# markokr/libacm

Hardware: AMD Instinct MI355X
Metric: decoded PCM Msamples/sec over a batch of ACM streams (hot path on HBM-resident staged input) (higher is better)
Workload: dtype int32

## Files before the change

libacm_amd/csrc/acm_kernel_geo.cpp:

```cpp
#include <stdlib.h>

#include "acm_kernel_geo.h"
#include "acm_parse_bounds.h"

using namespace acm_geo;

namespace {

inline int cus_of(int cus) { return cus > 0 ? cus : 256; }
inline int switch_of(const char *text, int unset) { return text ? atoi(text) : unset; }

inline const FusedTile *fused_at(uint32_t level, int variant)
{
	if (level < ACM_K1_MIN_LEVEL || level > ACM_K1_MAX_LEVEL || variant < 0 || variant >= NVARIANTS)
		return nullptr;
	return &FUSED[variant][level - ACM_K1_MIN_LEVEL];
}

const Tile2MTile *tile2m_at(uint32_t level, int *g0 = nullptr)
{
	if (level < ACM_K2M_MIN_LEVEL || level > ACM_K2M_MAX_LEVEL)
		return nullptr;
	static const bool k3 = switch_of(ACM_TUNING_ENV("ACM_K3"), 1) != 0;
	static const int forced = switch_of(ACM_TUNING_ENV("ACM_K2M_G0"), 0);
// ... 105 lines not shown

extern "C" int acmk_tile2m_stages(uint32_t level)
{
	int g0 = 0;
	return tile2m_at(level, &g0) ? g0 : 0;
}

extern "C" int acmk_tile2m_lead_in(uint32_t level)
{
	const Tile2MTile *m = tile2m_at(level);
	return m && m->t.nt ? m->lead_in : 1;
}

extern "C" int acmk_tile2m_run_waves(uint32_t level, int cus)
{
	const Tile2MTile *m = tile2m_at(level);
	return m && m->chunk ? cus_of(cus) * m->t.w * (m->t.nt / 64) : 0;
}

extern "C" int acmk_tile2m_grid(uint32_t level, int cus)
{
	const Tile2MTile *m = tile2m_at(level);
	return m ? cus_of(cus) * m->t.w : 0;
}

#define ACM_CLAIM_MIN_PER 32u
#ifndef ACM_CLAIM_DEFAULTS
#define ACM_CLAIM_DEFAULTS { 16, 900 }, { 16, 800 }, { 16, 800 }, { 16, 800 }, { 16, 900 }
#endif
static const struct { int run_chunks, static_permille; } g_claim_default[5] = { ACM_CLAIM_DEFAULTS };
static int g_claim_run_chunks = -1, g_claim_static_permille = -1;

extern "C" int acmk_tile2m_split(uint32_t level, int cus, uint32_t ntiles, uint32_t *static_per, uint32_t *run_chunks, uint32_t *nclaimed)
{
	const uint32_t W = (uint32_t)acmk_tile2m_run_waves(level, cus);
	if (!W)
		return -1;
	const bool set = g_claim_run_chunks >= 0 || g_claim_static_permille >= 0;
	const uint32_t R = (uint32_t)(g_claim_run_chunks >= 0 ? g_claim_run_chunks : g_claim_default[level - 8].run_chunks);
	uint32_t share = (uint32_t)(g_claim_static_permille >= 0 ? g_claim_static_permille : g_claim_default[level - 8].static_permille);
	if (share > 1000u)
		share = 1000u;
	*static_per = (ntiles + W - 1) / W;
	*run_chunks = *nclaimed = 0;
	if (!R || ntiles < (set ? (uint32_t)acmk_tile2m_grid(level, cus) : W * ACM_CLAIM_MIN_PER))
		return 0;
// ... 69 lines not shown
```

libacm_amd/csrc/acm_kernel_geo.h:

```cpp
#ifndef ACM_KERNEL_GEO_H
#define ACM_KERNEL_GEO_H

#include <stdint.h>

#include <initializer_list>

#include "acm_device.h"

#if defined(ACM_ABLATION) && !defined(ACM_TUNING)
#define ACM_TUNING 1
#endif

namespace acm_geo {

template <int L_, int NT_, int NELEM_>
struct TileCfg {
	static constexpr int L = L_;
	static constexpr int NT = NT_;
	static constexpr int NELEM = NELEM_;
	static constexpr int COLS = 1 << L_;
	static constexpr int TR = NELEM_ / COLS;
	static constexpr int NJ_LAST = NELEM_ / NT_;
	static constexpr int PS = NJ_LAST >= 64 ? 6 : 5;
	static_assert(NJ_LAST == 64 || NJ_LAST == 32 || NJ_LAST == 128, "walk length of the last pass");
	static_assert(TR >= 1, "whole rows");
	static constexpr bool ROW_PAIRS = TR >= 2 && (TR % 2) == 0;
};

struct Tile { int nt, nelem, w; };
struct Launch { int threads, tile_rows, wg_per_cu; };
constexpr Launch launch_of(const Tile t, const int level) { return Launch{ t.nt, t.nt ? t.nelem >> level : 0, t.w }; }

struct FusedTile { Tile t; bool carry = false; };
#ifdef ACM_ABLATION
constexpr int NVARIANTS = 20;
#elif defined(ACM_TUNING)
constexpr int NVARIANTS = 10;
#else
constexpr int NVARIANTS = 1;
#endif
constexpr FusedTile FUSED[NVARIANTS][ACM_K1_MAX_LEVEL - ACM_K1_MIN_LEVEL + 1] = {
	{ { { 128, 8192, 2 }, true }, { { 256, 16384, 2 }, true }, { { 256, 16384, 2 }, true }, { { 256, 16384, 2 }, true }, { { 256, 16384, 2 }, true },
	  { { 256, 16384, 2 }, true }, { { 512, 32768, 2 }, true }, { { 512, 32768, 2 }, true } },
#ifdef ACM_TUNING
	{ { { 128, 8192, 2 } }, { { 512, 16384, 4 } }, { { 512, 16384, 4 } }, { { 512, 16384, 4 } }, { { 512, 16384, 4 } }, { { 512, 32768, 2 } }, { { 512, 32768, 2 } } },
	{ { { 128, 8192, 2 } }, { { 512, 32768, 2 } }, { { 512, 32768, 2 } }, { { 512, 32768, 2 } }, { { 512, 32768, 2 } }, { { 512, 32768, 2 } }, { { 512, 32768, 2 } } },
// ... 26 lines not shown
constexpr FusedTile PLANE = { { 512, 32768, 2 }, true };
struct PlaneBuild {
	using C = TileCfg<12, PLANE.t.nt, PLANE.t.nelem>;
	static constexpr int W = PLANE.t.w;
};

constexpr Tile TILE2[ACM_K2_MAX_LEVEL - ACM_K2_MIN_LEVEL + 1] = {
	{ 256, 8192, 4 }, { 256, 8192, 4 }, { 256, 8192, 4 }, { 256, 8192, 4 }, { 256, 8192, 4 }, { 256, 8192, 4 },
	{ 512, 16384, 2 },
	{ 1024, 32768, 1 },
	{ 1024, 32768, 1 },
};
template <int L_, int NT_, int NELEM_, int WPC_>
struct TileBuildOf {
	using C = TileCfg<L_, NT_, NELEM_>;
	static constexpr int WPC = WPC_, W = WPC_ * NT_ / 256;
};
template <int L_>
struct Tile2Build : TileBuildOf<L_, TILE2[L_ - ACM_K2_MIN_LEVEL].nt, TILE2[L_ - ACM_K2_MIN_LEVEL].nelem, TILE2[L_ - ACM_K2_MIN_LEVEL].w> {};

#ifndef ACM_K3_DPP_HISTORY
#define ACM_K3_DPP_HISTORY 1
#endif
template <int L_>
struct ChunkGeo {
	static constexpr int NELEM = (1 << L_) > 2048 ? (1 << L_) : 2048;
	using C = TileCfg<L_, 64, NELEM>;
	static constexpr int NW = 32768 / NELEM;
	static constexpr int L = L_, COLS = C::COLS, TR = C::TR, PS = C::PS;
	static constexpr int G = 6, QN = 1 << G, SIGMA = COLS / QN;
	static_assert(SIGMA >= 2 && TR >= 1, "sixteen instances per matrix instruction: sixteen classes of one row, or all the classes of 2 / 4 / 8 rows");
	static constexpr int RR = SIGMA >= 16 ? 1 : 16 / SIGMA;
	static constexpr int NG = SIGMA >= 16 ? SIGMA / 16 : 1;
	static constexpr int NSW = TR / RR;
	static constexpr int NX = NSW + 2;
	static constexpr int NSET = NSW * NG;
	static constexpr int NE = (((TR & 1) + (RR - 1) * NSW + NX - 1) >> 1) + 1;
	static constexpr int NM = QN / 16;
	static_assert(NSW * RR == TR && NSET * 1024 == NELEM, "a chunk is whole sets");
	static constexpr bool HISTORY_IN_REGISTERS = RR == 1;
	static constexpr bool HISTORY_BY_DPP = ACM_K3_DPP_HISTORY && RR >= 2 && NSW == 2 && RR * SIGMA == 16 && SIGMA >= 4;
	static constexpr bool KEEPS_ROWS = HISTORY_IN_REGISTERS || HISTORY_BY_DPP;
	static constexpr Tile TILE = { 64 * NW, NELEM, 1 };
};

constexpr int lead_in_of(const bool keeps_rows, const int walk_rows) { return keeps_rows ? 1 + (2 + walk_rows - 1) / walk_rows : 1; }

struct Tile2MTile { Tile t; int lead_in; bool chunk; };
#ifdef ACM_TUNING
#define ACM_GEO_ALT(...) { { __VA_ARGS__ }, 1, false }
#else
#define ACM_GEO_ALT(...) { { 0, 0, 0 }, 1, false }
#endif
#ifndef ACM_K2M_L11_TILE
#define ACM_K2M_L11_TILE 256, 8192, 4
#endif
#ifndef ACM_K2M_L12_TILE
#define ACM_K2M_L12_TILE 512, 16384, 2
#endif
#ifndef ACM_K2M_L13_TILE
#define ACM_K2M_L13_TILE 512, 16384, 2
#endif
// ... 43 lines not shown
	static constexpr int NSLOT = (MAXCHUNKS + NW - 1) / NW;
	static constexpr int RS = C::COLS + (C::COLS >> C::PS);
	static_assert(GR % 4 == 0 && 64 % NQ == 0 && C::TR % GR == 0 && (P * NQ) % 64 == 0 && PERMB % 16 == 0, "packed geometry");
	static_assert(C::COLS % (1 << C::PS) == 0, "rows are whole pad groups");
};
template <int L_>
struct Tile2PBuild : TileBuildOf<L_, TILE2P[L_ - ACM_K2P_MIN_LEVEL].t.nt, TILE2P[L_ - ACM_K2P_MIN_LEVEL].t.nelem, TILE2P[L_ - ACM_K2P_MIN_LEVEL].t.w> {
	static constexpr int GR = TILE2P[L_ - ACM_K2P_MIN_LEVEL].gr;
	using PG = PackGeo<typename Tile2PBuild::C, GR>;
	static constexpr int SLOTS = PG::NW * PG::NSLOT, PAD_SHIFT = Tile2PBuild::C::PS;
};
struct PackSlots { int slots, pad_shift; };
template <int L_>
constexpr PackSlots pack_slots() { return PackSlots{ Tile2PBuild<L_>::SLOTS, Tile2PBuild<L_>::PAD_SHIFT }; }
constexpr PackSlots TILE2P_SLOTS[ACM_K2P_MAX_LEVEL - ACM_K2P_MIN_LEVEL + 1] = { pack_slots<6>(), pack_slots<7>(), pack_slots<8>(), pack_slots<9>() };

constexpr uint64_t mix(const uint64_t h, const int64_t v) { return (h ^ (uint64_t)v) * 0x100000001B3ull; }
constexpr uint64_t mix(const uint64_t h, const Tile t) { return mix(mix(mix(h, t.nt), t.nelem), t.w); }
template <int L_>
constexpr uint64_t mix_chunk(uint64_t h)
{
	using G = ChunkGeo<L_>;
	for (const int v : { G::NELEM, G::NW, G::TR, G::SIGMA, G::RR, G::NG, G::NSW, G::NX, G::NSET, G::NE, G::NM, (int)G::HISTORY_IN_REGISTERS,
			     (int)G::HISTORY_BY_DPP, (int)G::KEEPS_ROWS })
		h = mix(h, v);
	return h;
}
constexpr uint64_t digest()
{
	uint64_t h = 0xCBF29CE484222325ull;
	h = mix(h, NVARIANTS);
	for (const auto &row : FUSED)
		for (const FusedTile &f : row)
			h = mix(mix(h, f.t), f.carry);
	h = mix(mix(h, PLANE.t), PLANE.carry);
	for (const Tile &t : TILE2)
		h = mix(h, t);
	for (const auto &row : TILE2M)
		for (const Tile2MTile &m : row)
			h = mix(mix(mix(h, m.t), m.lead_in), m.chunk);
	for (const int g0 : TILE2M_DEFAULT_G0)
		h = mix(h, g0);
	h = mix_chunk<12>(mix_chunk<11>(mix_chunk<10>(mix_chunk<9>(mix_chunk<8>(h)))));
	for (const PackTile &p : TILE2P)
		h = mix(mix(h, p.t), p.gr);
	for (const PackSlots &p : TILE2P_SLOTS)
		h = mix(mix(h, p.slots), p.pad_shift);
// ... 7 lines not shown
```

libacm_amd/csrc/acm_kernels.hip:

```cpp
#include <hip/hip_runtime.h>

#include <utility>

#include "acm_device.h"
#include "acm_kernel_geo.h"

#ifndef ACM_L14_GROUPS
#define ACM_L14_GROUPS 3, 3, 3, 3, 2
#endif
#ifndef ACM_L13_GROUPS
#define ACM_L13_GROUPS 2, 3, 3, 3, 2
#endif

#ifndef ACM_OUT_F32
#define ACM_OUT_F32 0
#endif
#if ACM_OUT_F32
#define ACM_K_EMIT acm_sw_emit_f32
#define ACM_K_SMALL acm_small_level_f32
#define ACM_K_FUSED acm_fused_tile_f32
#define ACM_K_TILE2 acm_f32_tile2
#define ACM_K_CHUNK acm_f32_chunk
#define ACMK_OUT(name) name##_f32
#else
// ... 336 lines not shown
{
#define ACM_SDWA_MUL(D, S, WORD) "v_mul_i32_i24_sdwa " D ", sext(" S "), %12 dst_sel:DWORD dst_unused:UNUSED_PAD src0_sel:" WORD " src1_sel:DWORD\n\t"
	asm(ACM_SDWA_MUL("%0", "%8", "WORD_0") ACM_SDWA_MUL("%1", "%8", "WORD_1")
	    ACM_SDWA_MUL("%2", "%9", "WORD_0") ACM_SDWA_MUL("%3", "%9", "WORD_1")
	    ACM_SDWA_MUL("%4", "%10", "WORD_0") ACM_SDWA_MUL("%5", "%10", "WORD_1")
	    ACM_SDWA_MUL("%6", "%11", "WORD_0") ACM_SDWA_MUL("%7", "%11", "WORD_1")
	    : "=&v"(lo[0]), "=&v"(hi[0]), "=&v"(lo[1]), "=&v"(hi[1]), "=&v"(lo[2]), "=&v"(hi[2]), "=&v"(lo[3]), "=&v"(hi[3])
	    : "v"(r0), "v"(r1), "v"(r2), "v"(r3), "v"(val));
#undef ACM_SDWA_MUL
}

__device__ __forceinline__ uint32_t add_twice(uint32_t t, uint32_t z)
{
	uint32_t y;
	asm("v_lshl_add_u32 %0, %1, 1, %2" : "=v"(y) : "v"(z), "v"(t));
	return y;
}

template <int L, int K>
struct StageKind {
	static constexpr bool N = ((L - 1 - K) % 2) == 0;
};

template <int PS = 6>
__device__ __forceinline__ int lds_at(int m) { return m + (m >> PS); }
template <int NJ_LAST>
constexpr int park_piece() { return NJ_LAST == 32 ? 8 : 4; }

template <int L>
struct OutScale {
	static constexpr int SHIFT = (L <= 8) ? 8 - L : (L >= 10 ? 16 - L : 0);
	static constexpr int BYTE = (L <= 8) ? 1 : (L >= 10 ? 2 : 0);
	static constexpr bool PRESHIFT = (L == 9);
};

struct PcmFmt {
	uint32_t sel;
	uint32_t flip;
};

template <int L>
__device__ __forceinline__ PcmFmt make_pcm_fmt(unsigned fmt)
{
	PcmFmt f;
	const bool be = fmt & 1u, uns = fmt & 2u;
	constexpr uint32_t lo = OutScale<L>::BYTE, hi = OutScale<L>::BYTE + 1;
	f.sel = be ? ((4 + lo) << 24 | (4 + hi) << 16 | lo << 8 | hi)
		   : ((4 + hi) << 24 | (4 + lo) << 16 | hi << 8 | lo);
// ... 13 lines not shown
		}
		a >>= L;
		b >>= L;
	}
	const uint32_t p = __builtin_amdgcn_perm(b, a, f.sel);
	return FLIP ? (p ^ f.flip) : p;
}

template <class C, int K0, int G>
struct PassGeo {
	static constexpr int L = C::L;
	static constexpr int NT = C::NT;
	static constexpr int COLS = C::COLS;
	static constexpr int NELEM = C::NELEM;
	static constexpr int SIGMA = COLS >> (K0 + G);
	static constexpr int U = 1 << G;
	static constexpr int BODY = 2 * U;
	static constexpr int NJ_TOTAL = NELEM / SIGMA;
	static_assert(SIGMA < NT, "LDS passes need more threads than residues (the first pass takes the wide strides)");
	static constexpr int NSEG = NT / SIGMA;
	static constexpr int NJ = NJ_TOTAL / NSEG;
	static_assert(SIGMA >= 1, "pass exceeds level");
	static_assert(NJ % BODY == 0 && NJ >= BODY, "segment must be whole bodies");
	static constexpr int off(int u) { return u * SIGMA + ((u * SIGMA) >> C::PS); }
};

template <int L, int K0, int G>
__device__ __forceinline__ void pass_body(uint32_t (&v)[2 << G], uint32_t (&h)[G][1 << G],
					  uint32_t bias_lo, uint32_t bias_hi)
{
	constexpr int U = 1 << G, BODY = 2 * U;
	constexpr bool EXACT32 = (L > 9);
#pragma unroll
	for (int t = 0; t < G; t++) {
		const int d = 1 << (G - 1 - t);
		const int pb = G - 1 - t;
		const bool kindN = ((L - 1 - (K0 + t)) % 2) == 0;
		uint32_t in[BODY];
#pragma unroll
		for (int u = 0; u < BODY; u++)
			in[u] = v[u];
#pragma unroll
		for (int u = 0; u < BODY; u++) {
			const uint32_t z0 = in[u];
			const uint32_t z1 = (u >= d) ? in[u - d] : h[t][u + d];
			const uint32_t z2 = (u >= 2 * d) ? in[u - 2 * d] : h[t][u];
			const int beta = (u >> pb) & 1;
// ... 162 lines not shown
#pragma unroll
				for (int w = 0; w < W; w++)
#pragma unroll
					for (int u = 0; u < BODY; u++)
						v[w][u] = mul_idx_val<W == 2>(raw[(b + (WARM ? 1 : 0)) * BODY + u], u < U ? v0 : v1, w);
			}
#pragma unroll
			for (int w = 0; w < W; w++)
				if (!(ABL & 4))
					pass_body<L, 0, G>(v[w], h[w], w == 0 ? b0 : 0u, w == 0 ? b1 : 0u);
			if (b >= 0) {
				static_assert((2 * COLS) % 64 == 0 && (RPS * COLS) % 64 == 0, "row pairs are whole 64-element groups");
				uint32_t *o = tile + lds_at<C::PS>(lr_seg * COLS + i0) + b * (2 * COLS + ((2 * COLS) >> C::PS));
#pragma unroll
				for (int u = 0; u < BODY; u++)
#pragma unroll
					for (int w = 0; w < W; w++)
						o[off(u) + w] = v[w][u];
			}
		}
	}
};

constexpr int carry_words(int bs, int ps = 6) { return bs + (bs >> ps) + 2; }

template <class C, int K0, int G, bool LAST, int ABL = 0, bool FLIP = true, bool BIGEND = true, bool CARRY = false>
__device__ __forceinline__ void lds_pass(uint32_t *tile, const int tid, const unsigned fmt, uint32_t *carry = nullptr, const uint32_t bias = 0u,
					 const uint32_t bias_warm = 0u)
{
	using P = PassGeo<C, K0, G>;
	constexpr int L = C::L;
	constexpr int U = P::U, BODY = P::BODY, SIGMA = P::SIGMA;
	static_assert(!LAST || SIGMA == 1, "last pass must end at stride 1");

	const int seg = tid / SIGMA;
	const int i = tid % SIGMA;
	const int m_seg = seg * P::NJ * SIGMA + i;
	const PcmFmt pf = make_pcm_fmt<L>(fmt);
	constexpr int PS = C::PS, PG = 1 << PS;
	uint32_t *const base = tile + lds_at<PS>(m_seg);
	constexpr int BS = BODY * SIGMA;
	constexpr bool ALIGNED = (P::NJ * SIGMA) % PG == 0;
	auto body_ptr = [&](int it) -> uint32_t * {
		if constexpr (ALIGNED)
			return base + (it * BS + ((it * BS) >> PS));
		else
			return tile + lds_at<PS>(m_seg + it * BS);
	};
	uint32_t h[G][U];
	clear_hist<G>(h);

	tile_barrier<ABL>();
	uint32_t w[BODY];
	constexpr int NTAIL = CARRY ? (BS + C::NT - 1) / C::NT : 1;
	uint32_t tail[NTAIL];
	{
		const uint32_t *pw = ALIGNED ? base - (BS + (BS >= PG ? BS / PG : 1)) : tile + lds_at<PS>(m_seg - BS);
		if constexpr (CARRY) {
			if (seg == 0)
				pw = carry + i;
#pragma unroll
			for (int k = 0; k < NTAIL; k++) {
				const int j = tid + k * C::NT;
				tail[k] = (j < BS) ? tile[lds_at<PS>(C::NELEM - BS + j)] : 0u;
			}
		}
#pragma unroll
		for (int u = 0; u < BODY; u++)
			w[u] = pw[P::off(u)];
	}
	tile_barrier<ABL>();
	if constexpr (CARRY) {
#pragma unroll
		for (int k = 0; k < NTAIL; k++) {
			const int j = tid + k * C::NT;
			if (j < BS)
				carry[j + (((j / SIGMA) * SIGMA) >> PS)] = tail[k];
		}
	}

	constexpr int NBODY = P::NJ / BODY;
	uint32_t nxt[BODY];
	{
#pragma unroll
		for (int u = 0; u < BODY; u++)
			nxt[u] = base[P::off(u)];
	}
	if (!(ABL & 2))
		pass_body<L, K0, G>(w, h, K0 == 0 ? bias_warm : 0u, K0 == 0 ? bias_warm : 0u);

#pragma unroll
	for (int it = 0; it < NBODY; it++) {
		uint32_t *p = body_ptr(it);
		uint32_t v[BODY];
#pragma unroll
		for (int u = 0; u < BODY; u++)
			v[u] = nxt[u];
		if (it + 1 < NBODY && !(ABL & MODE_LEAN)) {
			const uint32_t *pn = body_ptr(it + 1);
#pragma unroll
			for (int u = 0; u < BODY; u++)
				nxt[u] = pn[P::off(u)];
		}
		if (!(ABL & 2))
			pass_body<L, K0, G>(v, h, K0 == 0 ? bias : 0u, K0 == 0 ? bias : 0u);
		if (it + 1 < NBODY && (ABL & MODE_LEAN) != 0) {
			__builtin_amdgcn_sched_barrier(0);
			const uint32_t *pn = body_ptr(it + 1);
#pragma unroll
			for (int u = 0; u < BODY; u++)
				nxt[u] = pn[P::off(u)];
		}
		if constexpr (!LAST) {
#pragma unroll
			for (int u = 0; u < BODY; u++)
				p[P::off(u)] = v[u];
		} else {
#pragma unroll
			for (int u = 0; u < BODY; u += 2) {
				const int d = it * (BODY / 2) + u / 2;
				base[(d / 4) * park_piece<C::NJ_LAST>() + d % 4] = pack_pcm<L, FLIP, BIGEND>(v[u], v[u + 1], pf);
			}
		}
	}
}

#ifdef ACM_STAMPS
__device__ unsigned long long g_acm_stamps[2048][8];
__device__ __forceinline__ unsigned long long stamp_now()
{
	unsigned long long t;
	__builtin_amdgcn_sched_barrier(0);
	asm volatile("s_memtime %0\n\ts_waitcnt lgkmcnt(0)" : "=s"(t) :: "memory");
	__builtin_amdgcn_sched_barrier(0);
	return t;
}
#define ACM_STAMP(k) do { const unsigned long long n_ = stamp_now(); acc_[k] += n_ - last_; last_ = n_; } while (0)
#define ACM_WAVE_STAMPS_MAX 8192
__device__ unsigned long long g_acm_wave_stamps[ACM_WAVE_STAMPS_MAX][8];
__device__ __forceinline__ void stamp_both(unsigned long long &shader, unsigned long long &real)
{
	__builtin_amdgcn_sched_barrier(0);
	asm volatile("s_memtime %0\n\ts_memrealtime %1\n\ts_waitcnt lgkmcnt(0)" : "=s"(shader), "=s"(real) :: "memory");
	__builtin_amdgcn_sched_barrier(0);
}
__device__ __forceinline__ unsigned long long stamp_where()
{
	uint32_t hw, xcc;
	asm volatile("s_getreg_b32 %0, hwreg(HW_REG_HW_ID)\n\ts_getreg_b32 %1, hwreg(HW_REG_XCC_ID)" : "=s"(hw), "=s"(xcc));
	return (unsigned long long)hw | (unsigned long long)xcc << 32;
}
#else
#define ACM_STAMP(k) do { } while (0)
#endif

template <class C, int K0, int G, int... Rest>
constexpr int carry_total()
{
	constexpr int mine = carry_words(PassGeo<C, K0, G>::BODY * PassGeo<C, K0, G>::SIGMA, C::PS);
	if constexpr (sizeof...(Rest) == 0)
		return mine;
	else
		return mine + carry_total<C, K0 + G, Rest...>();
}

template <class C, int ABL, bool CARRY, int K0, int G, int... Rest>
__device__ __forceinline__ void run_lds_passes(uint32_t *tile, int tid, unsigned fmt, uint32_t *carry = nullptr, const uint32_t bias = 0u,
					       const uint32_t bias_warm = 0u)
{
	constexpr bool last = sizeof...(Rest) == 0;
	static_assert(!last || K0 + G == C::L, "stage groups must add up to the level");
	uint32_t *cb = CARRY ? carry : nullptr;
	if constexpr (!last) {
		lds_pass<C, K0, G, false, ABL, true, true, CARRY>(tile, tid, fmt, cb, bias, bias_warm);
		run_lds_passes<C, ABL, CARRY, K0 + G, Rest...>(tile, tid, fmt,
							       CARRY ? carry + carry_words(PassGeo<C, K0, G>::BODY * PassGeo<C, K0, G>::SIGMA, C::PS) : nullptr);
	} else if (fmt == ACMHIP_FMT_S16LE) {
		lds_pass<C, K0, G, true, ABL, false, false, CARRY>(tile, tid, fmt, cb);
	} else {
		lds_pass<C, K0, G, true, ABL, true, true, CARRY>(tile, tid, fmt, cb);
	}
}

template <bool ON, int P>
__device__ __forceinline__ void phase_prio()
{
	if constexpr (ON)
		__builtin_amdgcn_s_setprio(P);
}
#ifndef ACM_PRIO_FIRST
#define ACM_PRIO_FIRST 2
#endif
#ifndef ACM_PRIO_LDS
#define ACM_PRIO_LDS 3
#endif
constexpr int PRIO_IDLE = 0, PRIO_FIRST_PASS = ACM_PRIO_FIRST, PRIO_LDS_PASSES = ACM_PRIO_LDS;

template <class C, int WAVES_PER_SIMD, int ABL, int W0, bool CARRY, int G0, int... Gs>
__global__ void __launch_bounds__(C::NT, WAVES_PER_SIMD)
// ... 906 lines not shown
#pragma unroll
				for (int g = 0; g < NGW; g++)
					raw.hi[g][k] &= mask;
			}
			if (__builtin_expect(whole_rows == 0u, 1))
				run_t<true>(raw, tile, rowval, in_front, tid, t);
			else
				run_t<true, true>(raw, tile, rowval, in_front, tid, t, whole_rows);
		} else {
			run_t<false>(raw, tile, rowval, in_front, tid, t);
		}
	}
};

#if defined(__HIP_DEVICE_COMPILE__) && !defined(__gfx950__)
#error "acm_kernels.hip: gfx950 (MI355X) only - the hand-counted s_waitcnt vmcnt(N) of acm_tile2 assumes in-order vector memory returns"
#endif

template <class C, int NP, int NSTORE, int ABL>
__device__ __forceinline__ void lean_store_f32(const uint32_t *tile, const int lane, float *out)
{
	constexpr int NJ_LAST = C::NJ_LAST, PER_OWNER = NJ_LAST / 8;
	static_assert((NP / 2) % PER_OWNER == 0 && NJ_LAST % (1 << C::PS) == 0, "round k's LDS address is round 0's plus a constant");
	constexpr int DQ = (NP / 2 / PER_OWNER) * (NJ_LAST + (NJ_LAST >> C::PS));
	const int v0 = lane / 2;
	uint32_t qa = (uint32_t)(lds_at<C::PS>((v0 / PER_OWNER) * NJ_LAST) + (v0 % PER_OWNER) * park_piece<NJ_LAST>() + 2 * (lane & 1));
	uint32_t oa = (uint32_t)lane * 16u;
	asm volatile("" : "+v"(qa), "+v"(oa));
#pragma unroll
	for (int k = 0; k < 2 * NSTORE; k++) {
		const uint32_t *q = tile + qa + k * DQ;
		const uint32_t a = q[0], b = q[1];
		if ((ABL & 16) && a != 0x12345u)
			continue;
		v4f *o = reinterpret_cast<v4f *>(reinterpret_cast<char *>(out) + oa + (uint32_t)(k * NP * 16));
		__builtin_nontemporal_store(pcm_quad_f32(a, b), o);
		if (k % 2)
			__builtin_amdgcn_sched_barrier(0);
	}
}

template <int YOUNGER>
__device__ __forceinline__ void k2_wait()
{
	static_assert(YOUNGER >= 0 && YOUNGER < 64, "vmcnt is a 6-bit field");
	asm volatile("s_waitcnt vmcnt(%0)" :: "n"(YOUNGER) : "memory");
}

template <class C, int WPS, int ABL, bool MFORM, int G0, int... Gs>
// ... 374 lines not shown
	}
	static __device__ __forceinline__ int32_t opaque_v(int32_t v)
	{
		asm("" : "+v"(v));
		return v;
	}

	template <bool WORDS, bool FAST, bool NIB = false>
	static __device__ __forceinline__ void run_t(const Raw &raw, uint32_t *const tile, const Tables &t, const int lane, const uint32_t hvs,
						     const uint32_t in_front, const uint32_t sval, const bool wordu = false, const Desc *dd = nullptr,
						     const uint32_t odd = 0u, const bool nform = false)
	{
		static_assert(!NIB || (WORDS && FAST), "rows in N form are a fast-path matter; the general path takes them to bytes first");
		const v4i_t zero = { 0, 0, 0, 0 };
		const uint32_t h = (uint32_t)lane >> 4, qd = (uint32_t)lane & 15u;
		uint32_t c0[NH], rrd[NH];
		uint32_t o_lane[NH];
#pragma unroll
		for (int hf = 0; hf < NH; hf++) {
			const uint32_t i = 4u * h + (uint32_t)(hf * NVH);
			c0[hf] = RR == 1 ? class_of(i) : i % SIGMA;
			rrd[hf] = RR == 1 ? 0u : i / SIGMA;
			const uint32_t m_lane = rrd[hf] * (uint32_t)(NSW * COLS) + c0[hf] + (uint32_t)SIGMA * qd;
			o_lane[hf] = m_lane + (m_lane >> PS);
		}
		uint32_t bias_at[NSW][NH];
		int32_t val[NSW][NH], dv2[NSW][NH], dv1[NSW][NH];
		bool step2[NSW], step1[NSW];
		bool small[NSW];
#pragma unroll
		for (int s = 0; s < NSW; s++)
			small[s] = OutScale<L>::SHIFT == 0;
		if constexpr (FAST) {
#pragma unroll
			for (int s = 0; s < NSW; s++) {
				step2[s] = step1[s] = false;
				small[s] = true;
#pragma unroll
				for (int hf = 0; hf < NH; hf++)
					val[s][hf] = dv2[s][hf] = dv1[s][hf] = 0;
			}
		} else if constexpr (RR <= 2) {
			int32_t rowval[TR + 2];
#pragma unroll
			for (int k = 0; k < TR + 2; k++)
				rowval[k] = (int32_t)__builtin_amdgcn_readlane(hvs, k);
#pragma unroll
// ... 147 lines not shown
						yh[v] = __mul24(ha[v], wv[v / NVH]);
					if (step2[s]) {
#pragma unroll
						for (int v = 0; v < 4; v++)
							yh[v] += __mul24(h2[v], w2[v / NVH]);
					}
					if (step1[s]) {
#pragma unroll
						for (int v = 0; v < 4; v++)
							yh[v] += __mul24(h1[v], w1[v / NVH]);
					}
					const uint32_t hs = nform ? 4u : 8u;
#pragma unroll
					for (int v = 0; v < 4; v++)
						y[v] = (int32_t)(((uint32_t)opaque_v(yh[v]) << hs) + (uint32_t)y[v]);
					}
				joined:;
				}
				}
				static_assert(COLS % (1 << PS) == 0 && (SIGMA * 16) % (1 << PS) == 0 &&
					      (NG == 1 || (group_at(NG - 1) % (1 << PS) + CB + 7 < (1 << PS) && SIGMA % (1 << PS) == 0)), "address split");
#pragma unroll
				for (int hf = 0; hf < NH; hf++) {
					uint32_t *const o = tile + (o_lane[hf] + (uint32_t)((s * COLS + ((s * COLS) >> PS)) + (group_at(g) + (group_at(g) >> PS))));
#pragma unroll
					for (int v = 0; v < NVH; v++)
						o[v] = (uint32_t)y[hf * NVH + v];
				}
			}
			cf += 64;
#pragma unroll
			for (int hf = 0; hf < NH; hf++)
				o_lane[hf] += SIGMA * 16 + ((SIGMA * 16) >> PS);
		}
	}

	static __device__ __forceinline__ void run(Raw &raw, uint32_t *const tile, const Tables &t, const int lane_, const uint32_t hvs,
						   const Desc &d, const uint32_t in_front, const uint32_t odd, const uint32_t mode, const uint32_t sval,
						   const bool first)
	{
#ifdef ACM_K3_OPAQUE_LANE
		const int lane = opaque_v(lane_);
#else
		const int lane = lane_;
#endif
		const bool all_new = !KEEPS_ROWS || first;
		if (mode == 3u) {
#pragma unroll
			for (int k = 0; k < NX; k++)
				if (k >= 2 || all_new) {
#pragma unroll
					for (int g = 0; g < NG; g++)
						raw.hi[g][k] = expand_nib(raw.hi[g][k]);
				}
			if constexpr (HISTORY_BY_DPP)
				take_history_from_partner(raw);
// ... 53 lines not shown
					if ((entry_of(d, (TR & 1 ? odd : 0u) + rr * NSW + k) & 3u) == ACMHIP_BP_NIB12) {
#pragma unroll
						for (int g = 0; g < NG; g++)
							raw.hi[g][k] = shl4(raw.hi[g][k]);
					}
			}
		} else {
			run_t<false, false>(raw, tile, t, lane, hvs, in_front, 0u);
		}
	}
};

template <int L_, int ABL, int... Gs>
__global__ void __launch_bounds__(64 * FirstPassZ<L_>::NW, 1)
ACM_K_CHUNK(const AcmTile2 *__restrict__ tiles, const uint32_t ntiles, const int16_t *__restrict__ idx, const uint32_t *__restrict__ pairs,
	  const acmhip_blkhdr *__restrict__ hdr, int16_t *__restrict__ pcm, int16_t *__restrict__ sink, const unsigned fmt,
	  uint32_t *__restrict__ claim, const uint32_t static_per, const uint32_t run_chunks, const uint32_t nclaimed)
{
	constexpr bool F32 = ACM_OUT_F32;

	using FP = FirstPassZ<L_>;
	using C = typename FP::C;
	constexpr int L = L_, COLS = C::COLS, NELEM = C::NELEM, TR = C::TR, NJ_LAST = C::NJ_LAST, NW = FP::NW;
	constexpr int WTILE = 8 + NELEM + (NELEM >> C::PS);
	constexpr int NCARRY_WORDS = carry_total<C, FP::G, Gs...>();
	constexpr int PASS_ABL = ABL | MODE_WAVE | (FP::NG > 1 && NW == 16 ? MODE_LEAN : 0);

	__shared__ uint32_t tile_mem[NW][WTILE];
	__shared__ uint32_t carry_all[NW][NCARRY_WORDS];
	__shared__ typename FP::Tables tables;

	const int lane0 = threadIdx.x & 63;
	const uint32_t wave = __builtin_amdgcn_readfirstlane(threadIdx.x >> 6);
	FP::fill_tables(tables, threadIdx.x, NW * 64);

	enum { SPLIT_CLAIM_LO, SPLIT_CLAIM_HI, SPLIT_WRAP, SPLIT_NCLAIMED, SPLIT_NSTATIC, SPLIT_RUN_CHUNKS, SPLIT_NTILES, SPLIT_WORDS };
	__shared__ __attribute__((aligned(8))) uint32_t split_mem[SPLIT_WORDS + 1];
	const uint32_t nvw = gridDim.x * NW, vw = blockIdx.x * NW + wave;
	const uint32_t per = nclaimed ? static_per : (ntiles + nvw - 1) / nvw;
	const uint32_t nstatic = nclaimed ? nvw * static_per : ntiles;
	if (threadIdx.x == 0) {
		const uint64_t c = nclaimed ? reinterpret_cast<uint64_t>(claim) : 0ull;
		split_mem[SPLIT_CLAIM_LO] = (uint32_t)c;
		split_mem[SPLIT_CLAIM_HI] = (uint32_t)(c >> 32);
		split_mem[SPLIT_WRAP] = nclaimed + nvw - 1;
		split_mem[SPLIT_NCLAIMED] = nclaimed;
		split_mem[SPLIT_NSTATIC] = nstatic;
		split_mem[SPLIT_RUN_CHUNKS] = run_chunks;
		split_mem[SPLIT_NTILES] = ntiles;
	}
	__syncthreads();

	uint32_t *const tile = tile_mem[wave] + 8;
	uint32_t *const carry_mem = carry_all[wave];

	uint32_t t = vw * per;
	uint32_t t_end = t + per < nstatic ? t + per : nstatic;
	if (t >= t_end) {
		if (!nclaimed)
			return;
		uint32_t k = 0;
		if (lane0 == 0)
			k = atomicInc(claim, nclaimed + nvw - 1);
		k = __builtin_amdgcn_readfirstlane(k);
		if (k >= nclaimed)
			return;
		t = nstatic + k * run_chunks;
		t_end = t + run_chunks < ntiles ? t + run_chunks : ntiles;
	}
	auto claim_next = [&](uint32_t v, const uint32_t more) -> uint32_t {
		uint64_t exec_was, at;
		asm volatile("s_cmp_lg_u32 %[more], 0\n\ts_cbranch_scc1 .Lacm_cl_%=\n\t"
			     "s_mov_b64 %[was], exec\n\ts_mov_b64 exec, 1\n\t"
			     "v_mov_b32 %[v], %[lds]\n\t"
			     "ds_read_b64 %[at], %[v]\n\tds_read_b32 %[v], %[v] offset:8\n\t"
			     "s_waitcnt lgkmcnt(0)\n\t"
// ... 122 lines not shown
					FP::zero_history(raw);
				FP::template issue<true>(raw, arena, dnxt, lane, (nxt.flags & ACM_TILE_ODD) ? 1u : 0u, mode_nxt);
			} else {
				FP::template issue<false>(raw, arena, dnxt, lane, (nxt.flags & ACM_TILE_ODD) ? 1u : 0u, mode_nxt);
			}
			claimed = claim_next(claimed, more ? 1u : 0u);
			const AcmTile2 nx3 = record_at(t + 3);
			const typename FP::Desc dnx2 = FP::fetch_desc(pairs, nx2);
			const uint32_t sv_nx2 = val_of(nx2);
			ACM_STAMP(2);
			phase_prio<true, PRIO_LDS_PASSES>();
			run_lds_passes<C, PASS_ABL, true, FP::G, Gs...>(tile, lane, F32 ? (unsigned)ACMHIP_FMT_S16LE : fmt, carry_mem);
			tile_barrier<MODE_WAVE>();
			ACM_STAMP(3);
			if constexpr (F32) {
				float *out = discard ? reinterpret_cast<float *>(sink) : reinterpret_cast<float *>(pcm) + cur.pcm_off;
				lean_store_f32<C, 64, NSTORE, ABL>(tile, lane, out);
			} else {
				typedef uint32_t v4u __attribute__((ext_vector_type(4)));
				v4u *out = discard ? reinterpret_cast<v4u *>(sink) : reinterpret_cast<v4u *>(reinterpret_cast<uint16_t *>(pcm) + cur.pcm_off);
#pragma unroll
				for (int k = 0; k < NSTORE; k++) {
					const int vec = lane + k * 64;
					const uint32_t *q = tile + lds_at<C::PS>((vec / PER_OWNER) * NJ_LAST) + (vec % PER_OWNER) * park_piece<NJ_LAST>();
					const v4u o = { q[0], q[1], q[2], q[3] };
#ifdef ACM_K3_ST_MOD
					asm volatile("global_store_dwordx4 %0, %1, %2" ACM_K3_ST_MOD :: "v"((uint32_t)(vec * 16)), "v"(o), "s"(sgpr_u64(reinterpret_cast<uint64_t>(out))) : "memory");
#else
					__builtin_nontemporal_store(o, &out[vec]);
#endif
				}
			}
			ACM_STAMP(5);
			phase_prio<true, PRIO_IDLE>();
			k2_wait<F32 ? 2 * NSTORE : NSTORE>();
			ACM_STAMP(6);
			tile_barrier<MODE_WAVE>();
			if (!more)
				break;
			fresh = (nxt.flags & (ACM_TILE_FRESH | ACM_TILE_DISCARD)) != 0;
			discard = (nxt.flags & ACM_TILE_DISCARD) != 0;
			cur = nxt;
			dcur = dnxt;
			sv_cur = sv_nxt;
			mode_cur = mode_nxt;
			t = tn;
			nxt = nx2;
			dnxt = dnx2;
// ... 620 lines not shown
```

Measured before the change: 1.364 million.

## Pad LDS tiles with four dwords per walk to enable 128-bit LDS accesses

Adds a configurable pad width (1 or 4 dwords per walk) to the chunk-kernel LDS tile layout, defaulting to 4 at level 9. With 16-byte-aligned walks the first-pass stores, LDS pass body reads, parked PCM writes and the final store gather can use ds_read/write_b128 instead of scalar dword accesses. The aim is fewer LDS instructions and less issue overhead. The cost is a larger LDS footprint per tile and carry buffer, which could affect occupancy or bank-conflict patterns. It also adds geometry query exports, static asserts on LDS budget, and an asm-counting script.

```diff
diff --git a/libacm_amd/csrc/acm_kernel_geo.cpp b/libacm_amd/csrc/acm_kernel_geo.cpp
--- a/libacm_amd/csrc/acm_kernel_geo.cpp
+++ b/libacm_amd/csrc/acm_kernel_geo.cpp
@@ -151,6 +151,74 @@
 {
 	const Tile2MTile *m = tile2m_at(level);
 	return m ? cus_of(cus) * m->t.w : 0;
+}
+
+template <int L_>
+static void chunk_layout_of(int *out)
+{
+	using G = ChunkGeo<L_>;
+	const int v[11] = { G::PW, G::PS, G::NELEM, G::GUARD, G::TILE_WORDS, G::NW, G::CARRY_WORDS, G::TABLE_BYTES, G::SPLIT_BYTES, G::LDS_BYTES, LDS_PER_CU };
+	for (int k = 0; k < 11; k++)
+		out[k] = v[k];
+}
+
+extern "C" int acmk_chunk_lds_layout(uint32_t level, int *out)
+{
+	switch (level) {
+	case 8: chunk_layout_of<8>(out); return 0;
+	case 9: chunk_layout_of<9>(out); return 0;
+	case 10: chunk_layout_of<10>(out); return 0;
+	case 11: chunk_layout_of<11>(out); return 0;
+	case 12: chunk_layout_of<12>(out); return 0;
+	default: return -1;
+	}
+}
+
+template <int L_>
+static int chunk_at_of(const int m)
+{
+	using G = ChunkGeo<L_>;
+	if (m < -G::GUARD || m >= G::NELEM)
+		return -1;
+	return G::GUARD + (m < 0 ? m : G::C::at(m));
+}
+
+extern "C" int acmk_chunk_lds_at(uint32_t level, int m)
+{
+	switch (level) {
+	case 8: return chunk_at_of<8>(m);
+	case 9: return chunk_at_of<9>(m);
+	case 10: return chunk_at_of<10>(m);
+	case 11: return chunk_at_of<11>(m);
+	case 12: return chunk_at_of<12>(m);
+	default: return -1;
+	}
+}
+
+extern "C" int acmk_chunk_carry_at(uint32_t level, int pass, int j, int *stride, int *count, int *base)
+{
+	int lay[11];
+	if (acmk_chunk_lds_layout(level, lay) || pass < 0 || pass >= 3)
+		return -1;
+	const int pw = lay[0], ps = lay[1];
+	int k0 = 6, at = 0;
+	for (int n = 0;; n++) {
+		const int g = CHUNK_GROUPS[level - 8][n];
+		if (!g)
+			return -1;
+		const int sigma = (1 << level) >> (k0 + g), bs = (2 << g) * sigma;
+		if (n == pass) {
+			if (stride)
+				*stride = sigma;
+			if (count)
+				*count = bs;
+			if (base)
+				*base = at;
+			return j < 0 || j >= bs ? -1 : carry_at(j, sigma, ps, pw);
+		}
+		at += carry_words(bs, ps, pw);
+		k0 += g;
+	}
 }
 
 #define ACM_CLAIM_MIN_PER 32u
diff --git a/libacm_amd/csrc/acm_kernel_geo.h b/libacm_amd/csrc/acm_kernel_geo.h
--- a/libacm_amd/csrc/acm_kernel_geo.h
+++ b/libacm_amd/csrc/acm_kernel_geo.h
@@ -13,7 +13,7 @@
 
 namespace acm_geo {
 
-template <int L_, int NT_, int NELEM_>
+template <int L_, int NT_, int NELEM_, int PW_ = 1>
 struct TileCfg {
 	static constexpr int L = L_;
 	static constexpr int NT = NT_;
@@ -22,6 +22,10 @@
 	static constexpr int TR = NELEM_ / COLS;
 	static constexpr int NJ_LAST = NELEM_ / NT_;
 	static constexpr int PS = NJ_LAST >= 64 ? 6 : 5;
+	static constexpr int PW = PW_;
+	static_assert(PW_ == 1 || PW_ == 4, "one pad dword per walk, or four: walks that start on 16-byte boundaries");
+	static constexpr int pad(const int m) { return PW_ * (m >> PS); }
+	static constexpr int at(const int m) { return m + pad(m); }
 	static_assert(NJ_LAST == 64 || NJ_LAST == 32 || NJ_LAST == 128, "walk length of the last pass");
 	static_assert(TR >= 1, "whole rows");
 	static constexpr bool ROW_PAIRS = TR >= 2 && (TR % 2) == 0;
@@ -94,10 +98,25 @@
 #ifndef ACM_K3_DPP_HISTORY
 #define ACM_K3_DPP_HISTORY 1
 #endif
+#ifndef ACM_K3_PAD_WORDS
+#define ACM_K3_PAD_WORDS 1, 4, 1, 1, 1
+#endif
+constexpr int CHUNK_PAD_WORDS[5] = { ACM_K3_PAD_WORDS };
+constexpr int CHUNK_GROUPS[5][3] = { { 2, 0, 0 }, { 3, 0, 0 }, { 2, 2, 0 }, { 3, 2, 0 }, { 3, 3, 0 } };
+constexpr int carry_words(const int bs, const int ps = 6, const int pw = 1) { return pw == 1 ? bs + (bs >> ps) + 2 : (bs + pw * (bs >> ps) + 3) & ~3; }
+constexpr int carry_at(const int j, const int sigma, const int ps, const int pw) { return j + pw * (((j / sigma) * sigma) >> ps); }
+constexpr int chunk_carry_total(const int level, const int ps, const int pw, const int k0 = 6, const int n = 0)
+{
+	const int g = level >= 8 && level <= 12 && n < 3 ? CHUNK_GROUPS[level - 8][n] : 0;
+	return g == 0 ? 0 : carry_words((2 << g) * ((1 << level) >> (k0 + g)), ps, pw) + chunk_carry_total(level, ps, pw, k0 + g, n + 1);
+}
+constexpr int LDS_PER_CU = 160 * 1024;
+
 template <int L_>
 struct ChunkGeo {
 	static constexpr int NELEM = (1 << L_) > 2048 ? (1 << L_) : 2048;
-	using C = TileCfg<L_, 64, NELEM>;
+	static constexpr int PW = L_ >= 8 && L_ <= 12 ? CHUNK_PAD_WORDS[L_ >= 8 && L_ <= 12 ? L_ - 8 : 0] : 1;
+	using C = TileCfg<L_, 64, NELEM, PW>;
 	static constexpr int NW = 32768 / NELEM;
 	static constexpr int L = L_, COLS = C::COLS, TR = C::TR, PS = C::PS;
 	static constexpr int G = 6, QN = 1 << G, SIGMA = COLS / QN;
@@ -110,6 +129,13 @@
 	static constexpr int NE = (((TR & 1) + (RR - 1) * NSW + NX - 1) >> 1) + 1;
 	static constexpr int NM = QN / 16;
 	static_assert(NSW * RR == TR && NSET * 1024 == NELEM, "a chunk is whole sets");
+	static constexpr int GUARD = PW == 4 ? 4 : 8;
+	static constexpr int TILE_WORDS = PW == 4 ? GUARD + C::at(NELEM) - PW : GUARD + C::at(NELEM);
+	static_assert(TILE_WORDS >= GUARD + C::at(NELEM - 1) + 1 && (PW == 1 || TILE_WORDS % 4 == 0), "every element has its dword; tiles of whole 16-byte pieces");
+	static constexpr int CARRY_WORDS = chunk_carry_total(L_, PS, PW);
+	static constexpr int TABLE_BYTES = 3 * NM * 64 * 16 + 3 * 2 * QN * 4 + 3 * QN * 4, SPLIT_BYTES = 8 * 4;
+	static constexpr int LDS_BYTES = NW * (TILE_WORDS + CARRY_WORDS) * 4 + TABLE_BYTES + SPLIT_BYTES;
+	static_assert(L_ < 8 || L_ > 12 || LDS_BYTES <= LDS_PER_CU, "sixteen tiles (eight at level 12), their carries, the tables and the split words in 160 KB");
 	static constexpr bool HISTORY_IN_REGISTERS = RR == 1;
 	static constexpr bool HISTORY_BY_DPP = ACM_K3_DPP_HISTORY && RR >= 2 && NSW == 2 && RR * SIGMA == 16 && SIGMA >= 4;
 	static constexpr bool KEEPS_ROWS = HISTORY_IN_REGISTERS || HISTORY_BY_DPP;
@@ -199,7 +225,7 @@
 {
 	using G = ChunkGeo<L_>;
 	for (const int v : { G::NELEM, G::NW, G::TR, G::SIGMA, G::RR, G::NG, G::NSW, G::NX, G::NSET, G::NE, G::NM, (int)G::HISTORY_IN_REGISTERS,
-			     (int)G::HISTORY_BY_DPP, (int)G::KEEPS_ROWS })
+			     (int)G::HISTORY_BY_DPP, (int)G::KEEPS_ROWS, G::PW, G::GUARD, G::TILE_WORDS, G::CARRY_WORDS, G::LDS_BYTES })
 		h = mix(h, v);
 	return h;
 }
diff --git a/libacm_amd/csrc/acm_kernels.hip b/libacm_amd/csrc/acm_kernels.hip
--- a/libacm_amd/csrc/acm_kernels.hip
+++ b/libacm_amd/csrc/acm_kernels.hip
@@ -382,8 +382,14 @@
 	static constexpr bool N = ((L - 1 - K) % 2) == 0;
 };
 
-template <int PS = 6>
-__device__ __forceinline__ int lds_at(int m) { return m + (m >> PS); }
+template <int PS = 6, int PW = 1>
+__device__ __forceinline__ int lds_at(int m) { return m + PW * (m >> PS); }
+#ifndef ACM_K3_WIDE
+#define ACM_K3_WIDE 11
+#endif
+typedef uint32_t lds_v4u __attribute__((ext_vector_type(4)));
+__device__ __forceinline__ lds_v4u lds_read4(const uint32_t *p) { return *reinterpret_cast<const lds_v4u *>(__builtin_assume_aligned(p, 16)); }
+__device__ __forceinline__ void lds_write4(uint32_t *p, const lds_v4u v) { *reinterpret_cast<lds_v4u *>(__builtin_assume_aligned(p, 16)) = v; }
 template <int NJ_LAST>
 constexpr int park_piece() { return NJ_LAST == 32 ? 8 : 4; }
 
@@ -443,7 +449,25 @@
 	static constexpr int NJ = NJ_TOTAL / NSEG;
 	static_assert(SIGMA >= 1, "pass exceeds level");
 	static_assert(NJ % BODY == 0 && NJ >= BODY, "segment must be whole bodies");
-	static constexpr int off(int u) { return u * SIGMA + ((u * SIGMA) >> C::PS); }
+	static constexpr int off(int u) { return C::at(u * SIGMA); }
+	static constexpr bool WIDE = C::PW == 4 && (ACM_K3_WIDE & 2) && SIGMA == 1 && BODY % 4 == 0 && BODY <= (1 << C::PS);
+	static constexpr bool WIDE_PARK = C::PW == 4 && (ACM_K3_WIDE & 4) && SIGMA == 1 && BODY % 8 == 0;
+	static __device__ __forceinline__ void read_body(uint32_t (&v)[BODY], const uint32_t *p)
+	{
+		if constexpr (WIDE) {
+#pragma unroll
+			for (int u = 0; u < BODY; u += 4) {
+				const lds_v4u x = lds_read4(p + u);
+#pragma unroll
+				for (int k = 0; k < 4; k++)
+					v[u + k] = x[k];
+			}
+		} else {
+#pragma unroll
+			for (int u = 0; u < BODY; u++)
+				v[u] = p[off(u)];
+		}
+	}
 };
 
 template <int L, int K0, int G>
@@ -652,7 +676,7 @@
 	}
 };
 
-constexpr int carry_words(int bs, int ps = 6) { return bs + (bs >> ps) + 2; }
+using acm_geo::carry_words;
 
 template <class C, int K0, int G, bool LAST, int ABL = 0, bool FLIP = true, bool BIGEND = true, bool CARRY = false>
 __device__ __forceinline__ void lds_pass(uint32_t *tile, const int tid, const unsigned fmt, uint32_t *carry = nullptr, const uint32_t bias = 0u,
@@ -667,15 +691,15 @@
 	const int i = tid % SIGMA;
 	const int m_seg = seg * P::NJ * SIGMA + i;
 	const PcmFmt pf = make_pcm_fmt<L>(fmt);
-	constexpr int PS = C::PS, PG = 1 << PS;
-	uint32_t *const base = tile + lds_at<PS>(m_seg);
+	constexpr int PS = C::PS, PG = 1 << PS, PW = C::PW;
+	uint32_t *const base = tile + lds_at<PS, PW>(m_seg);
 	constexpr int BS = BODY * SIGMA;
 	constexpr bool ALIGNED = (P::NJ * SIGMA) % PG == 0;
 	auto body_ptr = [&](int it) -> uint32_t * {
 		if constexpr (ALIGNED)
-			return base + (it * BS + ((it * BS) >> PS));
+			return base + C::at(it * BS);
 		else
-			return tile + lds_at<PS>(m_seg + it * BS);
+			return tile + lds_at<PS, PW>(m_seg + it * BS);
 	};
 	uint32_t h[G][U];
 	clear_hist<G>(h);
@@ -685,19 +709,17 @@
 	constexpr int NTAIL = CARRY ? (BS + C::NT - 1) / C::NT : 1;
 	uint32_t tail[NTAIL];
 	{
-		const uint32_t *pw = ALIGNED ? base - (BS + (BS >= PG ? BS / PG : 1)) : tile + lds_at<PS>(m_seg - BS);
+		const uint32_t *pw = ALIGNED ? base - (BS + PW * (BS >= PG ? BS / PG : 1)) : tile + lds_at<PS, PW>(m_seg - BS);
 		if constexpr (CARRY) {
 			if (seg == 0)
 				pw = carry + i;
 #pragma unroll
 			for (int k = 0; k < NTAIL; k++) {
 				const int j = tid + k * C::NT;
-				tail[k] = (j < BS) ? tile[lds_at<PS>(C::NELEM - BS + j)] : 0u;
-			}
-		}
-#pragma unroll
-		for (int u = 0; u < BODY; u++)
-			w[u] = pw[P::off(u)];
+				tail[k] = (j < BS) ? tile[lds_at<PS, PW>(C::NELEM - BS + j)] : 0u;
+			}
+		}
+		P::read_body(w, pw);
 	}
 	tile_barrier<ABL>();
 	if constexpr (CARRY) {
@@ -705,17 +727,13 @@
 		for (int k = 0; k < NTAIL; k++) {
 			const int j = tid + k * C::NT;
 			if (j < BS)
-				carry[j + (((j / SIGMA) * SIGMA) >> PS)] = tail[k];
+				carry[acm_geo::carry_at(j, SIGMA, PS, PW)] = tail[k];
 		}
 	}
 
 	constexpr int NBODY = P::NJ / BODY;
 	uint32_t nxt[BODY];
-	{
-#pragma unroll
-		for (int u = 0; u < BODY; u++)
-			nxt[u] = base[P::off(u)];
-	}
+	P::read_body(nxt, base);
 	if (!(ABL & 2))
 		pass_body<L, K0, G>(w, h, K0 == 0 ? bias_warm : 0u, K0 == 0 ? bias_warm : 0u);
 
@@ -728,28 +746,35 @@
 			v[u] = nxt[u];
 		if (it + 1 < NBODY && !(ABL & MODE_LEAN)) {
 			const uint32_t *pn = body_ptr(it + 1);
-#pragma unroll
-			for (int u = 0; u < BODY; u++)
-				nxt[u] = pn[P::off(u)];
+			P::read_body(nxt, pn);
 		}
 		if (!(ABL & 2))
 			pass_body<L, K0, G>(v, h, K0 == 0 ? bias : 0u, K0 == 0 ? bias : 0u);
 		if (it + 1 < NBODY && (ABL & MODE_LEAN) != 0) {
 			__builtin_amdgcn_sched_barrier(0);
 			const uint32_t *pn = body_ptr(it + 1);
-#pragma unroll
-			for (int u = 0; u < BODY; u++)
-				nxt[u] = pn[P::off(u)];
+			P::read_body(nxt, pn);
 		}
 		if constexpr (!LAST) {
 #pragma unroll
 			for (int u = 0; u < BODY; u++)
 				p[P::off(u)] = v[u];
 		} else {
+			if constexpr (P::WIDE_PARK) {
+#pragma unroll
+				for (int u = 0; u < BODY; u += 8) {
+					lds_v4u x;
+#pragma unroll
+					for (int k = 0; k < 4; k++)
+						x[k] = pack_pcm<L, FLIP, BIGEND>(v[u + 2 * k], v[u + 2 * k + 1], pf);
+					lds_write4(base + (it * (BODY / 8) + u / 8) * park_piece<C::NJ_LAST>(), x);
+				}
+			} else {
 #pragma unroll
 			for (int u = 0; u < BODY; u += 2) {
 				const int d = it * (BODY / 2) + u / 2;
 				base[(d / 4) * park_piece<C::NJ_LAST>() + d % 4] = pack_pcm<L, FLIP, BIGEND>(v[u], v[u + 1], pf);
+			}
 			}
 		}
 	}
@@ -787,7 +812,7 @@
 template <class C, int K0, int G, int... Rest>
 constexpr int carry_total()
 {
-	constexpr int mine = carry_words(PassGeo<C, K0, G>::BODY * PassGeo<C, K0, G>::SIGMA, C::PS);
+	constexpr int mine = carry_words(PassGeo<C, K0, G>::BODY * PassGeo<C, K0, G>::SIGMA, C::PS, C::PW);
 	if constexpr (sizeof...(Rest) == 0)
 		return mine;
 	else
@@ -804,7 +829,7 @@
 	if constexpr (!last) {
 		lds_pass<C, K0, G, false, ABL, true, true, CARRY>(tile, tid, fmt, cb, bias, bias_warm);
 		run_lds_passes<C, ABL, CARRY, K0 + G, Rest...>(tile, tid, fmt,
-							       CARRY ? carry + carry_words(PassGeo<C, K0, G>::BODY * PassGeo<C, K0, G>::SIGMA, C::PS) : nullptr);
+							       CARRY ? carry + carry_words(PassGeo<C, K0, G>::BODY * PassGeo<C, K0, G>::SIGMA, C::PS, C::PW) : nullptr);
 	} else if (fmt == ACMHIP_FMT_S16LE) {
 		lds_pass<C, K0, G, true, ABL, false, false, CARRY>(tile, tid, fmt, cb);
 	} else {
@@ -1757,9 +1782,9 @@
 {
 	constexpr int NJ_LAST = C::NJ_LAST, PER_OWNER = NJ_LAST / 8;
 	static_assert((NP / 2) % PER_OWNER == 0 && NJ_LAST % (1 << C::PS) == 0, "round k's LDS address is round 0's plus a constant");
-	constexpr int DQ = (NP / 2 / PER_OWNER) * (NJ_LAST + (NJ_LAST >> C::PS));
+	constexpr int DQ = (NP / 2 / PER_OWNER) * C::at(NJ_LAST);
 	const int v0 = lane / 2;
-	uint32_t qa = (uint32_t)(lds_at<C::PS>((v0 / PER_OWNER) * NJ_LAST) + (v0 % PER_OWNER) * park_piece<NJ_LAST>() + 2 * (lane & 1));
+	uint32_t qa = (uint32_t)(lds_at<C::PS, C::PW>((v0 / PER_OWNER) * NJ_LAST) + (v0 % PER_OWNER) * park_piece<NJ_LAST>() + 2 * (lane & 1));
 	uint32_t oa = (uint32_t)lane * 16u;
 	asm volatile("" : "+v"(qa), "+v"(oa));
 #pragma unroll
@@ -2180,7 +2205,7 @@
 			c0[hf] = RR == 1 ? class_of(i) : i % SIGMA;
 			rrd[hf] = RR == 1 ? 0u : i / SIGMA;
 			const uint32_t m_lane = rrd[hf] * (uint32_t)(NSW * COLS) + c0[hf] + (uint32_t)SIGMA * qd;
-			o_lane[hf] = m_lane + (m_lane >> PS);
+			o_lane[hf] = m_lane + C::PW * (m_lane >> PS);
 		}
 		uint32_t bias_at[NSW][NH];
 		int32_t val[NSW][NH], dv2[NSW][NH], dv1[NSW][NH];
@@ -2374,16 +2399,21 @@
 					      (NG == 1 || (group_at(NG - 1) % (1 << PS) + CB + 7 < (1 << PS) && SIGMA % (1 << PS) == 0)), "address split");
 #pragma unroll
 				for (int hf = 0; hf < NH; hf++) {
-					uint32_t *const o = tile + (o_lane[hf] + (uint32_t)((s * COLS + ((s * COLS) >> PS)) + (group_at(g) + (group_at(g) >> PS))));
+					uint32_t *const o = tile + (o_lane[hf] + (uint32_t)(C::at(s * COLS) + C::at((int)group_at(g))));
+					if constexpr (C::PW == 4 && NVH == 4 && (ACM_K3_WIDE & 1)) {
+						const lds_v4u x = { (uint32_t)y[0], (uint32_t)y[1], (uint32_t)y[2], (uint32_t)y[3] };
+						lds_write4(o, x);
+					} else {
 #pragma unroll
 					for (int v = 0; v < NVH; v++)
 						o[v] = (uint32_t)y[hf * NVH + v];
+					}
 				}
 			}
 			cf += 64;
 #pragma unroll
 			for (int hf = 0; hf < NH; hf++)
-				o_lane[hf] += SIGMA * 16 + ((SIGMA * 16) >> PS);
+				o_lane[hf] += C::at(SIGMA * 16);
 		}
 	}
 
@@ -2483,13 +2513,16 @@
 	using FP = FirstPassZ<L_>;
 	using C = typename FP::C;
 	constexpr int L = L_, COLS = C::COLS, NELEM = C::NELEM, TR = C::TR, NJ_LAST = C::NJ_LAST, NW = FP::NW;
-	constexpr int WTILE = 8 + NELEM + (NELEM >> C::PS);
+	using Geo = typename FP::Geo;
+	constexpr int WTILE = Geo::TILE_WORDS;
 	constexpr int NCARRY_WORDS = carry_total<C, FP::G, Gs...>();
+	static_assert(NCARRY_WORDS == Geo::CARRY_WORDS, "the LDS passes acm_kernel_geo.h counts the carry buffers of (CHUNK_GROUPS) are not the ones built here");
 	constexpr int PASS_ABL = ABL | MODE_WAVE | (FP::NG > 1 && NW == 16 ? MODE_LEAN : 0);
 
-	__shared__ uint32_t tile_mem[NW][WTILE];
-	__shared__ uint32_t carry_all[NW][NCARRY_WORDS];
+	__shared__ __attribute__((aligned(16))) uint32_t tile_mem[NW][WTILE];
+	__shared__ __attribute__((aligned(16))) uint32_t carry_all[NW][NCARRY_WORDS];
 	__shared__ typename FP::Tables tables;
+	static_assert(sizeof(typename FP::Tables) == Geo::TABLE_BYTES, "acm_kernel_geo.h counts the tables into a CU's LDS");
 
 	const int lane0 = threadIdx.x & 63;
 	const uint32_t wave = __builtin_amdgcn_readfirstlane(threadIdx.x >> 6);
@@ -2497,6 +2530,8 @@
 
 	enum { SPLIT_CLAIM_LO, SPLIT_CLAIM_HI, SPLIT_WRAP, SPLIT_NCLAIMED, SPLIT_NSTATIC, SPLIT_RUN_CHUNKS, SPLIT_NTILES, SPLIT_WORDS };
 	__shared__ __attribute__((aligned(8))) uint32_t split_mem[SPLIT_WORDS + 1];
+	static_assert(sizeof(split_mem) == Geo::SPLIT_BYTES && sizeof(tile_mem) + sizeof(carry_all) + sizeof(tables) + sizeof(split_mem) == Geo::LDS_BYTES &&
+		      Geo::LDS_BYTES <= acm_geo::LDS_PER_CU, "a CU's 160 KB hold every wavefront's tile and carries, the tables and the split words");
 	const uint32_t nvw = gridDim.x * NW, vw = blockIdx.x * NW + wave;
 	const uint32_t per = nclaimed ? static_per : (ntiles + nvw - 1) / nvw;
 	const uint32_t nstatic = nclaimed ? nvw * static_per : ntiles;
@@ -2512,7 +2547,7 @@
 	}
 	__syncthreads();
 
-	uint32_t *const tile = tile_mem[wave] + 8;
+	uint32_t *const tile = tile_mem[wave] + Geo::GUARD;
 	uint32_t *const carry_mem = carry_all[wave];
 
 	uint32_t t = vw * per;
@@ -2681,8 +2716,12 @@
 #pragma unroll
 				for (int k = 0; k < NSTORE; k++) {
 					const int vec = lane + k * 64;
-					const uint32_t *q = tile + lds_at<C::PS>((vec / PER_OWNER) * NJ_LAST) + (vec % PER_OWNER) * park_piece<NJ_LAST>();
-					const v4u o = { q[0], q[1], q[2], q[3] };
+					const uint32_t *q = tile + lds_at<C::PS, C::PW>((vec / PER_OWNER) * NJ_LAST) + (vec % PER_OWNER) * park_piece<NJ_LAST>();
+					v4u o;
+					if constexpr (C::PW == 4 && (ACM_K3_WIDE & 8))
+						o = lds_read4(q);
+					else
+						o = v4u{ q[0], q[1], q[2], q[3] };
 #ifdef ACM_K3_ST_MOD
 					asm volatile("global_store_dwordx4 %0, %1, %2" ACM_K3_ST_MOD :: "v"((uint32_t)(vec * 16)), "v"(o), "s"(sgpr_u64(reinterpret_cast<uint64_t>(out))) : "memory");
 #else
diff --git a/profiles/count_ds.py b/profiles/count_ds.py
--- /dev/null
+++ b/profiles/count_ds.py
@@ -0,0 +1,37 @@
+#!/usr/bin/env python3
+import collections
+import re
+import sys
+
+
+def main():
+    asm, level = open(sys.argv[1]).read(), sys.argv[2]
+    m = re.search(r"^(_ZN\S*acm_chunkILi%sE\S*):" % level, asm, re.M)
+    if not m:
+        raise SystemExit("no acm_chunk<%s> in %s" % (level, sys.argv[1]))
+    lines = asm[m.end():asm.index(".Lfunc_end", m.end())].split("\n")
+    base = asm[:m.end()].count("\n")
+    blocks, label, cur, start, n = [], "entry", collections.Counter(), 0, 0
+    for i, line in enumerate(lines):
+        t = line.split(";")[0].strip()
+        mm = re.fullmatch(r"(\.L\w+):", t)
+        if mm:
+            blocks.append((label, start, n, cur))
+            label, cur, start, n = mm.group(1), collections.Counter(), i, 0
+            continue
+        if not t or t.startswith("."):
+            continue
+        n += 1
+        if t.startswith("ds_"):
+            cur[t.split()[0]] += 1
+    blocks.append((label, start, n, cur))
+    total = collections.Counter()
+    for label, start, n, c in blocks:
+        total.update(c)
+        if c:
+            print("%-14s line %7d  insts %4d  %s" % (label, base + start + 1, n, " ".join("%s x%d" % kv for kv in sorted(c.items()))))
+    print("total %d: %s" % (sum(total.values()), " ".join("%s x%d" % kv for kv in sorted(total.items()))))
+
+
+if __name__ == "__main__":
+    main()
```

After: 1.372 million (median of 6 runs). No clear change (+0.6%).
